# zjykzj/YOLOv4

Hardware: AMD Instinct MI355X
Metric: images/sec fwd+bwd @608x608 bs=64 per GPU (YOLOv4 training step: forward + YOLOLoss + backward) (higher is better)
Workload: dtype f32

## Files before the change

include/yolov4_amd.h:

```cpp
#ifndef YOLOV4_AMD_H
#define YOLOV4_AMD_H

#include <stddef.h>
#include <stdint.h>

#ifdef __cplusplus
extern "C" {
#endif

#define Y4_OK 0
#define Y4_ERR_SHAPE 1
#define Y4_ERR_NULL 2
#define Y4_ERR_LAUNCH 3
#define Y4_ERR_WORKSPACE 4
#define Y4_ERR_NODEVICE 5
#define Y4_ERR_FORMAT 6
#define Y4_ERR_UNSUPPORTED 7

#define Y4_ACT_LINEAR 0
#define Y4_ACT_LEAKY 1
#define Y4_ACT_MISH 2
#define Y4_ACT_RELU 3

const char* y4_strerror(int code);
// ... 75 lines not shown
size_t y4_conv2d_dgrad_workspace(int Cin, int Cout, int k);
int y4_conv2d_dgrad_f32(const float* dy, int lddy, const float* w , float* dx, int lddx,
                        int B, int H, int W, int Cin, int Cout, int k, int stride,
                        void* workspace, size_t workspace_bytes, const unsigned* dy_amax ,
                        const float* residual, int ldr, void* stream);

size_t y4_conv2d_wgrad_workspace(int B, int H, int W, int Cin, int Cout, int k, int stride);
int y4_conv2d_wgrad_f32(const float* x, int ldx, const float* dy, int lddy, float* dw,
                        int B, int H, int W, int Cin, int Cout, int k, int stride,
                        void* workspace, size_t workspace_bytes,
                        const unsigned* x_amax, const unsigned* dy_amax , void* stream);
size_t y4_conv2d_stem_wgrad_workspace(int B, int H, int W, int Cout);
int y4_conv2d_stem_wgrad_f32(const float* x, long long sxb, long long sxc, long long sxh, long long sxw,
                             const float* dy, int lddy, float* dw, int B, int H, int W, int Cout,
                             void* workspace, size_t workspace_bytes, void* stream);

size_t y4_bn_workspace(long long M, int C);
size_t y4_bn_finalize_workspace(int C);
int y4_bn_stats_f32(const float* y, int ldy, long long M, int C, float* mean, float* invstd,
                    float* running_mean, float* running_var, long long* num_batches_tracked,
                    float momentum, float eps, void* workspace, size_t workspace_bytes, void* stream);
int y4_bn_finalize_partials_f32(const float* partials, long long nparts, long long M, int C,
                                float* mean, float* invstd, float* running_mean, float* running_var,
                                long long* num_batches_tracked, float momentum, float eps,
                                void* workspace, size_t workspace_bytes, void* stream);
int y4_bn_planes_bound_f32(const float* gamma, const float* beta, int C, long long M, const unsigned* floor_word, unsigned* out,
                           void* stream);
int y4_bn_act_fwd_f32(const float* y, int ldy, const float* mean, const float* invstd,
                      const float* gamma, const float* beta, int act,
                      const float* residual, int ldr, float* z, int ldz,
// ... 190 lines not shown
```

yolov4_amd/_lib.py:

```python
import ctypes
import os
from ctypes import c_char_p, c_double, c_float, c_int, c_longlong, c_size_t, c_void_p

_HERE = os.path.dirname(os.path.abspath(__file__))
LIB_PATH = os.environ.get('Y4_LIB_PATH') or os.path.join(_HERE, 'lib', 'libyolov4_amd.so')

ACT_IDS = {'linear': 0, 'leaky_relu': 1, 'mish': 2, 'relu': 3}


class Y4Error(RuntimeError):
    pass


P = c_void_p
I, L, F, Z = c_int, c_longlong, c_float, c_size_t

PROTOTYPES = {
    'y4_strerror': (c_char_p, [I]),
    'y4_version': (I, []),
    'y4_device_count': (I, []),
    'y4_set_conv_mode': (I, [I]),
    'y4_get_conv_mode': (I, []),
    'y4_set_planes_bf16': (I, [I]),
    'y4_get_planes_bf16': (I, []),
# ... 13 lines not shown
    'y4_conv2d_fwd_planes_f32': (I, [P, P, P, I, I, I, I, I, I, I, I, P, Z, P, P, P, Z, P, Z, I, P, P]),
    'y4_conv2d_dgrad_planes_f32': (I, [P, P, P, I, I, I, I, I, I, I, I, P, Z, P, P, I, P]),
    'y4_conv2d_wgrad_planes_workspace': (Z, [I, I, I, I, I, I, I]),
    'y4_conv2d_wgrad_planes_f32': (I, [P, P, P, I, I, I, I, I, I, I, P, Z, P, P, P]),
    'y4_conv2d_generic_fwd_f32': (I, [P, I, P, P, I, I, I, I, I, I, I, I, P, P, I, P, I, P]),
    'y4_conv2d_generic_dgrad_f32': (I, [P, I, P, P, I, I, I, I, I, I, I, I, P, I, P]),
    'y4_conv2d_generic_wgrad_f32': (I, [P, I, P, I, P, I, I, I, I, I, I, I, P]),
    'y4_conv2d_stem_dgrad_f32': (I, [P, I, P, P, L, L, L, L, I, I, I, I, P]),
    'y4_conv2d_stem_fwd_f32': (I, [P, L, L, L, L, P, P, I, I, I, I, I, P, P, I, P, P]),
    'y4_conv2d_dgrad_workspace': (Z, [I, I, I]),
    'y4_conv2d_dgrad_f32': (I, [P, I, P, P, I, I, I, I, I, I, I, I, P, Z, P, P, I, P]),
    'y4_conv2d_wgrad_workspace': (Z, [I, I, I, I, I, I, I]),
    'y4_conv2d_wgrad_f32': (I, [P, I, P, I, P, I, I, I, I, I, I, I, P, Z, P, P, P]),
    'y4_conv2d_stem_wgrad_workspace': (Z, [I, I, I, I]),
    'y4_conv2d_stem_wgrad_f32': (I, [P, L, L, L, L, P, I, P, I, I, I, I, P, Z, P]),
    'y4_bn_workspace': (Z, [L, I]),
    'y4_bn_finalize_workspace': (Z, [I]),
    'y4_bn_finalize_partials_f32': (I, [P, L, L, I, P, P, P, P, P, F, F, P, Z, P]),
    'y4_bn_stats_f32': (I, [P, I, L, I, P, P, P, P, P, F, F, P, Z, P]),
    'y4_bn_act_fwd_f32': (I, [P, I, P, P, P, P, I, P, I, P, I, L, I, P, I, P, P, P]),
    'y4_bn_planes_bound_f32': (I, [P, P, I, L, P, P, P]),
    'y4_bn_act_bwd_f32': (I, [P, I, P, I, P, P, P, P, I, P, I, P, P, L, I, P, Z, P, P, P, I, P]),
    'y4_bias_grad_workspace': (Z, [L, I]),
    'y4_bias_grad_f32': (I, [P, I, L, I, P, P, Z, P]),
    'y4_bn_fold_f32': (I, [P, P, P, P, F, P, P, I, P]),
    'y4_copy_channels_f32': (I, [P, I, P, I, L, I, P]),
    'y4_add_f32': (I, [P, I, P, I, P, I, L, I, P]),
    'y4_maxpool_s1_fwd_f32': (I, [P, I, P, I, P, I, I, I, I, I, P]),
    'y4_maxpool_s1_bwd_f32': (I, [P, I, P, P, I, I, I, I, I, I, I, P]),
    'y4_upsample2x_fwd_f32': (I, [P, I, P, I, I, I, I, I, P]),
# ... 110 lines not shown
```

yolov4_amd/csrc/common.h:

```cpp
#pragma once
#include <hip/hip_runtime.h>
#include <stdint.h>
#include "../../include/yolov4_amd.h"

typedef float f32x4 __attribute__((ext_vector_type(4)));
typedef float f32x16 __attribute__((ext_vector_type(16)));
typedef unsigned int u32x4 __attribute__((ext_vector_type(4)));

#define Y4_CHECK_LAUNCH()                                   \
    do {                                                    \
        if (hipGetLastError() != hipSuccess) return Y4_ERR_LAUNCH; \
    } while (0)

static inline hipStream_t y4_stream(void* s) { return reinterpret_cast<hipStream_t>(s); }

#include <atomic>
struct Y4DynLds {
    std::atomic<unsigned long long> done{0ull};
    bool ensure(const void* kernel, size_t bytes) {
        int d = 0;
        if (hipGetDevice(&d) != hipSuccess) return false;
        if (d >= 0 && d < 64 && ((done.load(std::memory_order_acquire) >> d) & 1ull)) return true;
        if (hipFuncSetAttribute(kernel, hipFuncAttributeMaxDynamicSharedMemorySize, (int)bytes) != hipSuccess) return false;
        if (d >= 0 && d < 64) done.fetch_or(1ull << d, std::memory_order_release);
// ... 51 lines not shown
}

__device__ __forceinline__ int y4_xcd_remap(int bid, int nwg) {
    const int q = nwg >> 3, r = nwg & 7, xcd = bid & 7;
    const int base = (xcd < r) ? xcd * (q + 1) : r * (q + 1) + (xcd - r) * q;
    return base + (bid >> 3);
}

__device__ __forceinline__ __amdgpu_buffer_rsrc_t y4_make_rsrc(const void* base, unsigned num_bytes) {
    return __builtin_amdgcn_make_buffer_rsrc(const_cast<void*>(base), (short)0, (int)num_bytes, 0x00020000);
}
__device__ __forceinline__ f32x4 y4_buf_load4(__amdgpu_buffer_rsrc_t r, unsigned voff_bytes, unsigned soff_bytes) {
    const u32x4 v = __builtin_amdgcn_raw_buffer_load_b128(r, (int)voff_bytes, (int)soff_bytes, 0);
    return __builtin_bit_cast(f32x4, v);
}
```

yolov4_amd/csrc/conv_igemm.hip:

```cpp
#include <stdlib.h>
#include "common.h"
#include <cstdarg>
#include <cstdio>
#include "conv_geom.h"

namespace {

constexpr int BK = 32;


using y4::ConvGeom;
using y4::WgradGeom;

template <int BM, int BN, int WM, int WN, bool TRANSPOSED, int BKT = 32>
__global__ __launch_bounds__(256, (BKT == 16 ? 3 : 2)) void conv_gather_mfma_f32(const ConvGeom g) {
    constexpr int LPR = BKT / 4;
    constexpr int RPP = 256 / LPR;
    constexpr int PA = BM / RPP, PB = BN / RPP;
    constexpr int LDS_PITCH = BKT + 4;
    constexpr int BK = BKT;
    constexpr int WTM = BM / WM, WTN = BN / WN;
    constexpr int TM = WTM / 32, TN = WTN / 32;
    static_assert(WM * WN == 4, "4 waves");
    extern __shared__ __attribute__((aligned(16))) float smem[];
// ... 214 lines not shown
        }
        __syncthreads();
        for (int c = tid; c < BN; c += 256) {
            float cs = 0.f, css = 0.f;
#pragma unroll
            for (int w = 0; w < WM; ++w) { cs += red[(w * BN + c) * 2]; css += red[(w * BN + c) * 2 + 1]; }
            const int n = n0 + c;
            if (n < g.N) {
                g.stats[((long long)mt_local * 2 + 0) * g.N + n] = cs;
                g.stats[((long long)mt_local * 2 + 1) * g.N + n] = css;
            }
        }
    }
}

typedef __bf16 bf16x8 __attribute__((ext_vector_type(8)));
typedef unsigned int u32x2 __attribute__((ext_vector_type(2)));

__device__ __forceinline__ unsigned pack_hi16(unsigned x1, unsigned x0) { return __builtin_amdgcn_perm(x1, x0, 0x07060302u); }

__device__ __forceinline__ unsigned rn_bf16_bits(float x) {
    const unsigned u = __float_as_uint(x);
    return u + 0x7fffu + ((u >> 16) & 1u);
}
__device__ __forceinline__ u32x2 round1x4(const f32x4 v) {
    u32x2 p;
    p[0] = pack_hi16(rn_bf16_bits(v[1]), rn_bf16_bits(v[0]));
    p[1] = pack_hi16(rn_bf16_bits(v[3]), rn_bf16_bits(v[2]));
    return p;
}

__device__ __forceinline__ void split3x4(const f32x4 v, u32x2& p1, u32x2& p2, u32x2& p3) {
    unsigned h1[4], h2[4], h3[4];
#pragma unroll
    for (int e = 0; e < 4; ++e) {
        h1[e] = __float_as_uint(v[e]);
        const float r1 = v[e] - __uint_as_float(h1[e] & 0xffff0000u);
        h2[e] = __float_as_uint(r1);
        const float r2 = r1 - __uint_as_float(h2[e] & 0xffff0000u);
        h3[e] = __float_as_uint(r2);
    }
    p1[0] = pack_hi16(h1[1], h1[0]); p1[1] = pack_hi16(h1[3], h1[2]);
    p2[0] = pack_hi16(h2[1], h2[0]); p2[1] = pack_hi16(h2[3], h2[2]);
    p3[0] = pack_hi16(h3[1], h3[0]); p3[1] = pack_hi16(h3[3], h3[2]);
}

template <int BM, int BN, int WM, int WN, bool TRANSPOSED, int NP = 3>
__global__ __launch_bounds__(256, 2) void conv_gather_bf16x3(const ConvGeom g) {
    constexpr int BK = 32;
    constexpr int PITCH_B = 80;
    constexpr int PA = BM / 32;
    constexpr int NB = (BN * 4 + 255) / 256;
    constexpr int WTM = BM / WM, WTN = BN / WN;
    constexpr int TM = WTM / 32, TN = WTN / 32;
    static_assert(WM * WN == 4, "4 waves");
    extern __shared__ __attribute__((aligned(16))) unsigned char smem_b[];
    unsigned char* As = smem_b;
    unsigned char* Bs = smem_b + NP * BM * PITCH_B;
    int* row_m = reinterpret_cast<int*>(smem_b + NP * (BM + BN) * PITCH_B);
// ... 1288 lines not shown
__global__ __launch_bounds__(256) void stem_wgrad_reduce2_kernel(const double* __restrict__ part, float* __restrict__ dw,
                                                                 int nparts, int Cout) {
    for (int i = threadIdx.x; i < Cout * 27; i += 256) {
        const int n = i / 27, j = i - n * 27;
        double s = 0.0;
        for (int k = 0; k < nparts; ++k) s += part[(long long)k * 1024 + n * 32 + j];
        dw[i] = (float)s;
    }
}

constexpr int STEM_WAVES = 4096;

}

namespace y4 {
int slab_reduce(const float* slabs, float* dw, long long n, int splits, hipStream_t st) {
    if ((n & 3) == 0 && !(reinterpret_cast<uintptr_t>(dw) & 15) && !(reinterpret_cast<uintptr_t>(slabs) & 15)) {
        const long long nvec = n / 4;
        if (nvec >= 64 * 1024)
            hipLaunchKernelGGL(slab_reduce_vec_kernel<64>, dim3((unsigned)((nvec + 63) / 64)), dim3(256), 0, st,
                               reinterpret_cast<const f32x4*>(slabs), reinterpret_cast<f32x4*>(dw), nvec, splits);
        else
            hipLaunchKernelGGL(slab_reduce_vec_kernel<16>, dim3((unsigned)((nvec + 15) / 16)), dim3(256), 0, st,
                               reinterpret_cast<const f32x4*>(slabs), reinterpret_cast<f32x4*>(dw), nvec, splits);
    } else {
        const int blocks = (int)((n + 255) / 256 > 2048 ? 2048 : (n + 255) / 256);
        hipLaunchKernelGGL(slab_reduce_kernel, dim3(blocks), dim3(256), 0, st, slabs, dw, n, splits);
    }
    Y4_CHECK_LAUNCH();
    return Y4_OK;
// ... 381 lines not shown
```

yolov4_amd/csrc/pointwise.hip:

```cpp
#include "common.h"

namespace {

constexpr int PW_THREADS = 256;
constexpr int PW_UNROLL = 4;
#define Y4_ACT_SWITCH(ACTV, CALL)                                              \
    switch (ACTV) {                                                            \
        case Y4_ACT_MISH: { constexpr int A_ = Y4_ACT_MISH; CALL; } break;     \
        case Y4_ACT_LEAKY: { constexpr int A_ = Y4_ACT_LEAKY; CALL; } break;   \
        case Y4_ACT_RELU: { constexpr int A_ = Y4_ACT_RELU; CALL; } break;     \
        default: { constexpr int A_ = Y4_ACT_LINEAR; CALL; } break;            \
    }

struct RowMap {
    int tpr;
    int rpb;
};
static inline RowMap row_map(int C) {
    RowMap r;
    int c4 = C / 4;
    r.tpr = c4 < PW_THREADS ? c4 : PW_THREADS;
    int p = 1;
    while (p * 2 <= r.tpr) p *= 2;
    r.tpr = p;
// ... 132 lines not shown
    if (blockIdx.x == 0 && threadIdx.x == 0 && nbt) *nbt += 1;
    const int c = blockIdx.x * 32 + (threadIdx.x & 31);
    if ((threadIdx.x >> 5) != 0 || c >= C) return;
    const double mu = s / (double)M;
    double var = ss / (double)M - mu * mu;
    if (var < 0) var = 0;
    mean[c] = (float)mu;
    invstd[c] = (float)(1.0 / sqrt(var + (double)eps));
    if (rmean) rmean[c] = (1.0f - momentum) * rmean[c] + momentum * (float)mu;
    if (rvar) {
        const double unb = M > 1 ? var * (double)M / (double)(M - 1) : var;
        rvar[c] = (1.0f - momentum) * rvar[c] + momentum * (float)unb;
    }
}

__device__ __forceinline__ void amax_track(unsigned& m, const f32x4 o) {
#pragma unroll
    for (int e = 0; e < 4; ++e) {
        const unsigned b = __float_as_uint(o[e]) & 0x7fffffffu;
        if (b < 0x7f800000u && b > m) m = b;
    }
}
__device__ __forceinline__ void amax_commit(unsigned m, unsigned* out) {
    __shared__ unsigned wmax[PW_THREADS / 64];
#pragma unroll
    for (int off = 32; off > 0; off >>= 1) {
        const unsigned o = (unsigned)__shfl_xor((int)m, off, 64);
        m = o > m ? o : m;
    }
    if ((threadIdx.x & 63) == 0) wmax[threadIdx.x >> 6] = m;
    __syncthreads();
    if (threadIdx.x == 0) {
        unsigned v = wmax[0];
#pragma unroll
        for (int w = 1; w < PW_THREADS / 64; ++w) v = wmax[w] > v ? wmax[w] : v;
        if (v > __hip_atomic_load(out, __ATOMIC_RELAXED, __HIP_MEMORY_SCOPE_AGENT)) atomicMax(out, v);
    }
}

__global__ __launch_bounds__(256) void bn_planes_bound_kernel(const float* __restrict__ gamma, const float* __restrict__ beta, int C,
                                                              float sqrt_m1, const unsigned* __restrict__ res_amax,
                                                              unsigned* __restrict__ out, const unsigned* __restrict__ floor_word = nullptr) {
    __shared__ float red[256];
    float m = 0.f;
    for (int c = threadIdx.x; c < C; c += 256) m = fmaxf(m, fabsf(gamma[c]) * sqrt_m1 + fabsf(beta[c]));
    red[threadIdx.x] = m;
    __syncthreads();
    for (int s = 128; s > 0; s >>= 1) {
        if (threadIdx.x < s) red[threadIdx.x] = fmaxf(red[threadIdx.x], red[threadIdx.x + s]);
        __syncthreads();
    }
    if (threadIdx.x == 0) {
        float b = red[0] * 1.0001f;
// ... 944 lines not shown
    if (n <= 0 || act < 0 || act > 3) return Y4_ERR_SHAPE;
    hipLaunchKernelGGL(act_fwd_flat_kernel, dim3(grid_for((n + 3) / 4)), dim3(PW_THREADS), 0, y4_stream(stream), x, y, n, act);
    Y4_CHECK_LAUNCH();
    return Y4_OK;
}

int y4_act_bwd_f32(const float* x, const float* dy, float* dx, long long n, int act, void* stream) {
    if (!x || !dy || !dx) return Y4_ERR_NULL;
    if (n <= 0 || act < 0 || act > 3) return Y4_ERR_SHAPE;
    hipLaunchKernelGGL(act_bwd_flat_kernel, dim3(grid_for((n + 3) / 4)), dim3(PW_THREADS), 0, y4_stream(stream), x, dy, dx, n, act);
    Y4_CHECK_LAUNCH();
    return Y4_OK;
}

}
```

yolov4_amd/ops.py:

```python
import ctypes
import functools
import os

import torch

from ._lib import ACT_IDS, Y4Error, check, float_array, int_array, lib

CL = torch.channels_last


def _stream():
    return ctypes.c_void_p(torch.cuda.current_stream().cuda_stream)


def _ptr(t):
    return ctypes.c_void_p(t.data_ptr()) if t is not None else None


def _require_gpu(t, what):
    if not t.is_cuda:
        raise Y4Error(f'{what}: tensor is on {t.device}; the yolov4_amd hot path runs on an MI355X only '
                      '(no CPU fallback)')
    if t.dtype != torch.float32:
        raise Y4Error(f'{what}: expected float32, got {t.dtype}')
# ... 263 lines not shown
        nbytes = L.y4_conv2d_fwd_workspace(Cin, Cout, k)
        cws = _ws(nbytes, x.device)
        check(L.y4_conv2d_fwd_bnstats_f32(_ptr(x), ldx, _ptr(w), _ptr(y), ldy, B, H, W, Cin, Cout, k, s,
                                          _ptr(part), pbytes, ctypes.byref(n), _ptr(x_amax), _ptr(cws), nbytes,
                                          _ptr(dgrad_filter), dgrad_filter.numel() if dgrad_filter is not None else 0, _stream()),
              'conv2d_fwd_bnstats')
        nparts = n.value
    mean = torch.empty(Cout, device=x.device, dtype=torch.float32)
    invstd = torch.empty(Cout, device=x.device, dtype=torch.float32)
    wsb = L.y4_bn_finalize_workspace(Cout)
    ws = _ws(wsb, x.device)
    check(L.y4_bn_finalize_partials_f32(_ptr(part), nparts, B * Ho * Wo, Cout, _ptr(mean), _ptr(invstd),
                                        _ptr(running_mean), _ptr(running_var), _ptr(nbt), float(momentum), float(eps),
                                        _ptr(ws), wsb, _stream()), 'bn_finalize_partials')
    return y, mean, invstd


class Planes:
    __slots__ = ('buf', 'shape', 'amax')

    def __init__(self, buf, shape, amax):
        self.buf, self.shape, self.amax = buf, tuple(shape), amax


class PlanesTensor(torch.Tensor):
    __torch_function__ = torch._C._disabled_torch_function_impl

    def _refuse(self, *a, **kw):
        raise Y4Error('this tensor holds a PRE-SPLIT activation (two fp16 pieces per element, csrc/conv_planes.hip), not '
                      'float32 values: only ConvBNAct can consume it.  Register the forward hook before the forward pass '
# ... 455 lines not shown
        if xp is not None:
            x_amax = xp.amax
        elif f16 and x_amax is None and (ctx.needs_input_grad[0] or ctx.needs_input_grad[1]):
            x_amax = amax_raw(x)
        ctx.x_amax = x_amax
        if bn and training:
            if x.shape[0] * conv_out_hw(x.shape[2], x.shape[3], k, s)[0] * conv_out_hw(x.shape[2], x.shape[3], k, s)[1] <= 1:
                raise ValueError('Expected more than 1 value per channel when training')
            ctx.dgrad_filter = None
            if ((f16 or (bfm and xp is not None)) and ctx.needs_input_grad[0] and x.shape[1] % 32 == 0 and fast_conv_shape(x.shape[1], k, s)
                    and weight.shape[0] % 4 == 0 and (xp is None or weight.shape[0] % 32 == 0)
                    and not (bfm and xp is not None and s == 2
                             and not s2_plane_dgrad(x.shape[0], x.shape[2], x.shape[3], x.shape[1], weight.shape[0]))):
                ctx.dgrad_filter = dgrad_filter_buffer(x.shape[1], weight.shape[0], k, x.device)
            ybf = ctx.y_bf16 = bool(bfm and xp is not None and weight.shape[0] % 32 == 0 and _BF16_Y)
            if xp is not None:
                y, mean, invstd = conv_fwd_planes_bnstats_raw(xp, weight, k, s, cfg['running_mean'], cfg['running_var'],
                                                              cfg['nbt'], cfg['momentum'], cfg['eps'], dgrad_filter=ctx.dgrad_filter,
                                                              y_bf16=ybf)
            else:
                y, mean, invstd = conv_fwd_bnstats_raw(x, weight, k, s, cfg['running_mean'], cfg['running_var'],
                                                       cfg['nbt'], cfg['momentum'], cfg['eps'], x_amax=x_amax,
                                                       dgrad_filter=ctx.dgrad_filter)
            want = cfg.get('out_planes')
            cb = cfg.get('out_cat')
            if cb is not None and cb.planes:
                z = bn_act_fwd_raw(y, mean, invstd, gamma, beta, act, residual, out=dest, planes='slot', y_bf16=ybf)
                if io is not None:
                    io['z_planes'] = True
                z_amax = cb.cell[0:1] if cb.cell is not None else None
# ... 63 lines not shown
            else:
                ctx.save_for_backward(x, weight)
                ctx.mode = 'nobn_linear'
        if io is not None:
            io['z_amax'] = z_amax
        return z

    @staticmethod
    def backward(ctx, dz):
        cfg = ctx.cfg
        k, s, act = cfg['k'], cfg['s'], cfg['act']
        f16 = f16x2_mode() and ctx.x_shape[1] != 3
        dy_amax = dy_pl = dyP = wq = None
        x_amax = live(ctx.x_amax)
        x_planes = getattr(ctx, 'x_planes', False)
        if ctx.mode in ('bn_train', 'bn_eval_grad'):
            x, weight, y, mean, invstd, gamma, beta = ctx.saved_tensors
            gp, bp = cfg.get('gamma_param'), cfg.get('beta_param')
            sink = (gp is not None and bp is not None and getattr(gp, '_y4_grad_fresh', False)
                    and getattr(bp, '_y4_grad_fresh', False) and gp.grad is not None and bp.grad is not None
                    and ctx.needs_input_grad[3] and ctx.needs_input_grad[4])
            bfp = x_planes and planes_mode() == 'bf16'
            planes = planes_cell(dz.device, 8) if (x_planes and not bfp) else None
            dy_amax = planes[5:6] if planes is not None else (new_amax(dz.device) if f16 else None)
            twin_dy = x_planes and s == 2 and ctx.needs_input_grad[0] and not s2_plane_dgrad(
                ctx.x_shape[0], ctx.x_shape[2], ctx.x_shape[3], ctx.x_shape[1], dz.shape[1])
            res = bn_act_bwd_raw(dz, y, mean, invstd, gamma, beta, act,
                                 gp.grad if sink else None, bp.grad if sink else None,
                                 out_amax=None if planes is not None else dy_amax, planes=planes,
                                 frozen=ctx.mode == 'bn_eval_grad', bf16=bfp, twin=twin_dy, y_bf16=getattr(ctx, 'y_bf16', False))
# ... 731 lines not shown
```

Measured before the change: 449.0.

## Fuse stem conv with BatchNorm and activation via recompute in fwd and bwd

Adds a dedicated stem path (3-channel 3x3 stride-1 conv) that runs the conv with bf16x3 split MFMA, first to compute BN statistics and then again to apply BN+activation and write z directly, so the pre-BN y tensor is never stored. The backward pass recomputes the conv output to get BN/activation gradients and fuses the weight gradient into the same pass, with no dgrad since the input needs no gradient. This removes a full-resolution read and write of y at 608x608 with 32 channels. The cost is doing the conv two or three times, plus new kernels and several extra small reduction launches.

```diff
diff --git a/include/yolov4_amd.h b/include/yolov4_amd.h
--- a/include/yolov4_amd.h
+++ b/include/yolov4_amd.h
@@ -113,6 +113,19 @@
 int y4_conv2d_stem_wgrad_f32(const float* x, long long sxb, long long sxc, long long sxh, long long sxw,
                              const float* dy, int lddy, float* dw, int B, int H, int W, int Cout,
                              void* workspace, size_t workspace_bytes, void* stream);
+
+int y4_stem_fused_ok(long long sxb, long long sxc, long long sxh, long long sxw, int B, int H, int W, int Cout);
+size_t y4_stem_bn_act_fwd_workspace(int B, int H, int W, int Cout);
+int y4_stem_bn_act_fwd_f32(const float* x, long long sxb, long long sxc, long long sxh, long long sxw, const float* w,
+                           int B, int H, int W, int Cout, const float* gamma, const float* beta, int act,
+                           float* mean, float* invstd, float* running_mean, float* running_var, long long* num_batches_tracked,
+                           float momentum, float eps, float* z, int ldz, unsigned* out_amax,
+                           void* workspace, size_t workspace_bytes, void* stream);
+size_t y4_stem_bn_act_bwd_workspace(int B, int H, int W, int Cout);
+int y4_stem_bn_act_bwd_f32(const float* x, long long sxb, long long sxc, long long sxh, long long sxw, const float* w,
+                           const float* dz, int lddz, const float* mean, const float* invstd, const float* gamma,
+                           const float* beta, int act, int B, int H, int W, int Cout,
+                           float* dgamma, float* dbeta, float* dw, void* workspace, size_t workspace_bytes, void* stream);
 
 size_t y4_bn_workspace(long long M, int C);
 size_t y4_bn_finalize_workspace(int C);
diff --git a/yolov4_amd/_lib.py b/yolov4_amd/_lib.py
--- a/yolov4_amd/_lib.py
+++ b/yolov4_amd/_lib.py
@@ -51,6 +51,11 @@
     'y4_conv2d_wgrad_f32': (I, [P, I, P, I, P, I, I, I, I, I, I, I, P, Z, P, P, P]),
     'y4_conv2d_stem_wgrad_workspace': (Z, [I, I, I, I]),
     'y4_conv2d_stem_wgrad_f32': (I, [P, L, L, L, L, P, I, P, I, I, I, I, P, Z, P]),
+    'y4_stem_fused_ok': (I, [L, L, L, L, I, I, I, I]),
+    'y4_stem_bn_act_fwd_workspace': (Z, [I, I, I, I]),
+    'y4_stem_bn_act_fwd_f32': (I, [P, L, L, L, L, P, I, I, I, I, P, P, I, P, P, P, P, P, F, F, P, I, P, P, Z, P]),
+    'y4_stem_bn_act_bwd_workspace': (Z, [I, I, I, I]),
+    'y4_stem_bn_act_bwd_f32': (I, [P, L, L, L, L, P, P, I, P, P, P, P, I, I, I, I, I, P, P, P, P, Z, P]),
     'y4_bn_workspace': (Z, [L, I]),
     'y4_bn_finalize_workspace': (Z, [I]),
     'y4_bn_finalize_partials_f32': (I, [P, L, L, I, P, P, P, P, P, F, F, P, Z, P]),
diff --git a/yolov4_amd/csrc/common.h b/yolov4_amd/csrc/common.h
--- a/yolov4_amd/csrc/common.h
+++ b/yolov4_amd/csrc/common.h
@@ -89,3 +89,52 @@
     const u32x4 v = __builtin_amdgcn_raw_buffer_load_b128(r, (int)voff_bytes, (int)soff_bytes, 0);
     return __builtin_bit_cast(f32x4, v);
 }
+
+typedef __bf16 bf16x8 __attribute__((ext_vector_type(8)));
+typedef unsigned int u32x2 __attribute__((ext_vector_type(2)));
+__device__ __forceinline__ unsigned pack_hi16(unsigned x1, unsigned x0) { return __builtin_amdgcn_perm(x1, x0, 0x07060302u); }
+__device__ __forceinline__ void split3x4(const f32x4 v, u32x2& p1, u32x2& p2, u32x2& p3) {
+    unsigned h1[4], h2[4], h3[4];
+#pragma unroll
+    for (int e = 0; e < 4; ++e) {
+        h1[e] = __float_as_uint(v[e]);
+        const float r1 = v[e] - __uint_as_float(h1[e] & 0xffff0000u);
+        h2[e] = __float_as_uint(r1);
+        const float r2 = r1 - __uint_as_float(h2[e] & 0xffff0000u);
+        h3[e] = __float_as_uint(r2);
+    }
+    p1[0] = pack_hi16(h1[1], h1[0]); p1[1] = pack_hi16(h1[3], h1[2]);
+    p2[0] = pack_hi16(h2[1], h2[0]); p2[1] = pack_hi16(h2[3], h2[2]);
+    p3[0] = pack_hi16(h3[1], h3[0]); p3[1] = pack_hi16(h3[3], h3[2]);
+}
+
+__device__ __forceinline__ void amax_track1(unsigned& m, const float o) {
+    const unsigned b = __float_as_uint(o) & 0x7fffffffu;
+    if (b < 0x7f800000u && b > m) m = b;
+}
+__device__ __forceinline__ void amax_track(unsigned& m, const f32x4 o) {
+#pragma unroll
+    for (int e = 0; e < 4; ++e) amax_track1(m, o[e]);
+}
+__device__ __forceinline__ void amax_commit(unsigned m, unsigned* out) {
+    __shared__ unsigned wmax[4];
+#pragma unroll
+    for (int off = 32; off > 0; off >>= 1) {
+        const unsigned o = (unsigned)__shfl_xor((int)m, off, 64);
+        m = o > m ? o : m;
+    }
+    if ((threadIdx.x & 63) == 0) wmax[threadIdx.x >> 6] = m;
+    __syncthreads();
+    if (threadIdx.x == 0) {
+        unsigned v = wmax[0];
+#pragma unroll
+        for (int w = 1; w < 4; ++w) v = wmax[w] > v ? wmax[w] : v;
+        if (v > __hip_atomic_load(out, __ATOMIC_RELAXED, __HIP_MEMORY_SCOPE_AGENT)) atomicMax(out, v);
+    }
+}
+
+namespace y4 {
+int bn_bwd_fold_finalize(const float* part, long long nparts, long long M, int C, void* workspace, float* dgamma, float* dbeta,
+                         const float* gamma, const float* invstd, hipStream_t st);
+int stem_wgrad_fold(const float* slabs, int nslabs, double* part, float* dw, int Cout, hipStream_t st);
+}
diff --git a/yolov4_amd/csrc/conv_igemm.hip b/yolov4_amd/csrc/conv_igemm.hip
--- a/yolov4_amd/csrc/conv_igemm.hip
+++ b/yolov4_amd/csrc/conv_igemm.hip
@@ -252,10 +252,6 @@
     }
 }
 
-typedef __bf16 bf16x8 __attribute__((ext_vector_type(8)));
-typedef unsigned int u32x2 __attribute__((ext_vector_type(2)));
-
-__device__ __forceinline__ unsigned pack_hi16(unsigned x1, unsigned x0) { return __builtin_amdgcn_perm(x1, x0, 0x07060302u); }
 
 __device__ __forceinline__ unsigned rn_bf16_bits(float x) {
     const unsigned u = __float_as_uint(x);
@@ -266,21 +262,6 @@
     p[0] = pack_hi16(rn_bf16_bits(v[1]), rn_bf16_bits(v[0]));
     p[1] = pack_hi16(rn_bf16_bits(v[3]), rn_bf16_bits(v[2]));
     return p;
-}
-
-__device__ __forceinline__ void split3x4(const f32x4 v, u32x2& p1, u32x2& p2, u32x2& p3) {
-    unsigned h1[4], h2[4], h3[4];
-#pragma unroll
-    for (int e = 0; e < 4; ++e) {
-        h1[e] = __float_as_uint(v[e]);
-        const float r1 = v[e] - __uint_as_float(h1[e] & 0xffff0000u);
-        h2[e] = __float_as_uint(r1);
-        const float r2 = r1 - __uint_as_float(h2[e] & 0xffff0000u);
-        h3[e] = __float_as_uint(r2);
-    }
-    p1[0] = pack_hi16(h1[1], h1[0]); p1[1] = pack_hi16(h1[3], h1[2]);
-    p2[0] = pack_hi16(h2[1], h2[0]); p2[1] = pack_hi16(h2[3], h2[2]);
-    p3[0] = pack_hi16(h3[1], h3[0]); p3[1] = pack_hi16(h3[3], h3[2]);
 }
 
 template <int BM, int BN, int WM, int WN, bool TRANSPOSED, int NP = 3>
@@ -1599,6 +1580,13 @@
 }
 
 namespace y4 {
+int stem_wgrad_fold(const float* slabs, int nslabs, double* part, float* dw, int Cout, hipStream_t st) {
+    hipLaunchKernelGGL(stem_wgrad_reduce1_kernel, dim3(64), dim3(256), 0, st, slabs, part, nslabs);
+    Y4_CHECK_LAUNCH();
+    hipLaunchKernelGGL(stem_wgrad_reduce2_kernel, dim3(1), dim3(256), 0, st, part, dw, 64, Cout);
+    Y4_CHECK_LAUNCH();
+    return Y4_OK;
+}
 int slab_reduce(const float* slabs, float* dw, long long n, int splits, hipStream_t st) {
     if ((n & 3) == 0 && !(reinterpret_cast<uintptr_t>(dw) & 15) && !(reinterpret_cast<uintptr_t>(slabs) & 15)) {
         const long long nvec = n / 4;
diff --git a/yolov4_amd/csrc/pointwise.hip b/yolov4_amd/csrc/pointwise.hip
--- a/yolov4_amd/csrc/pointwise.hip
+++ b/yolov4_amd/csrc/pointwise.hip
@@ -170,29 +170,6 @@
     }
 }
 
-__device__ __forceinline__ void amax_track(unsigned& m, const f32x4 o) {
-#pragma unroll
-    for (int e = 0; e < 4; ++e) {
-        const unsigned b = __float_as_uint(o[e]) & 0x7fffffffu;
-        if (b < 0x7f800000u && b > m) m = b;
-    }
-}
-__device__ __forceinline__ void amax_commit(unsigned m, unsigned* out) {
-    __shared__ unsigned wmax[PW_THREADS / 64];
-#pragma unroll
-    for (int off = 32; off > 0; off >>= 1) {
-        const unsigned o = (unsigned)__shfl_xor((int)m, off, 64);
-        m = o > m ? o : m;
-    }
-    if ((threadIdx.x & 63) == 0) wmax[threadIdx.x >> 6] = m;
-    __syncthreads();
-    if (threadIdx.x == 0) {
-        unsigned v = wmax[0];
-#pragma unroll
-        for (int w = 1; w < PW_THREADS / 64; ++w) v = wmax[w] > v ? wmax[w] : v;
-        if (v > __hip_atomic_load(out, __ATOMIC_RELAXED, __HIP_MEMORY_SCOPE_AGENT)) atomicMax(out, v);
-    }
-}
 
 __global__ __launch_bounds__(256) void bn_planes_bound_kernel(const float* __restrict__ gamma, const float* __restrict__ beta, int C,
                                                               float sqrt_m1, const unsigned* __restrict__ res_amax,
@@ -1167,3 +1144,18 @@
 }
 
 }
+
+namespace y4 {
+int bn_bwd_fold_finalize(const float* part, long long nparts, long long M, int C, void* workspace, float* dgamma, float* dbeta,
+                         const float* gamma, const float* invstd, hipStream_t st) {
+    double* acc = static_cast<double*>(workspace);
+    double* bacc = acc + 2 * C;
+    int nb = 0;
+    const int rc = fold_partials(part, nparts, C, bacc, &nb, st);
+    if (rc != Y4_OK) return rc;
+    hipLaunchKernelGGL(bn_bwd_finalize_kernel, dim3((C + 31) / 32), dim3(256), 0, st, bacc, nb, C, acc, dgamma, dbeta, gamma,
+                       invstd, 1.0 / (double)M, static_cast<unsigned*>(nullptr));
+    Y4_CHECK_LAUNCH();
+    return Y4_OK;
+}
+}
diff --git a/yolov4_amd/csrc/stem_fused.hip b/yolov4_amd/csrc/stem_fused.hip
--- /dev/null
+++ b/yolov4_amd/csrc/stem_fused.hip
@@ -0,0 +1,423 @@
+#include "conv_geom.h"
+
+namespace {
+
+struct StemFusedGeom {
+    const float* x; const float* w;
+    long long sxb, sxc, sxh, sxw;
+    int B, H, W, Cout;
+    long long M;
+    int ngroups;
+    float inv_hw, inv_w;
+    const float* mean; const float* invstd; const float* gamma; const float* beta;
+    float* stats;
+    float* z; long long ldz; unsigned* out_amax;
+    const float* dz; long long lddz;
+    float* part;
+    const double* acc; double invM;
+    float* slabs;
+};
+
+struct StemBody {
+    bf16x8 fb[2][3];
+    int koff[16];
+    int ktap[16];
+    __amdgpu_buffer_rsrc_t rsrc;
+
+    __device__ __forceinline__ void init(const StemFusedGeom& g, int fr, int fh) {
+#pragma unroll
+        for (int i = 0; i < 16; ++i) {
+            const int k = (i >> 3) * 16 + fh * 8 + (i & 7);
+            const int r = k / 9, c = (k - r * 9) / 3, q = k - r * 9 - c * 3;
+            const bool kv = k < 27;
+            koff[i] = kv ? (int)(c * g.sxc + (r - 1) * g.sxh + (q - 1) * g.sxw) * 4 : 0;
+            ktap[i] = kv ? r * 3 + q : 9;
+        }
+#pragma unroll
+        for (int ks = 0; ks < 2; ++ks) {
+            f32x4 w0, w1;
+#pragma unroll
+            for (int i = 0; i < 8; ++i) {
+                const int k = ks * 16 + fh * 8 + i;
+                const int r = k / 9, c = (k - r * 9) / 3, q = k - r * 9 - c * 3;
+                const float v = (k < 27 && fr < g.Cout) ? g.w[fr * 27 + (r * 3 + q) * 3 + c] : 0.f;
+                if (i < 4) w0[i] = v; else w1[i - 4] = v;
+            }
+            u32x2 a1, a2, a3, b1, b2, b3;
+            split3x4(w0, a1, a2, a3);
+            split3x4(w1, b1, b2, b3);
+            const u32x4 q1 = {a1[0], a1[1], b1[0], b1[1]}, q2 = {a2[0], a2[1], b2[0], b2[1]}, q3 = {a3[0], a3[1], b3[0], b3[1]};
+            fb[ks][0] = __builtin_bit_cast(bf16x8, q1); fb[ks][1] = __builtin_bit_cast(bf16x8, q2); fb[ks][2] = __builtin_bit_cast(bf16x8, q3);
+        }
+        rsrc = y4_make_rsrc(g.x, 0xfffffff0u);
+    }
+
+    static __device__ __forceinline__ void coords(const StemFusedGeom& g, long long p, int& b, int& h, int& w) {
+        const int HW = g.H * g.W;
+        b = (int)((float)p * g.inv_hw);
+        int rem = (int)(p - (long long)b * HW);
+        if (rem < 0) { --b; rem += HW; } else if (rem >= HW) { ++b; rem -= HW; }
+        h = (int)((float)rem * g.inv_w);
+        w = rem - h * g.W;
+        if (w < 0) { --h; w += g.W; } else if (w >= g.W) { ++h; w -= g.W; }
+    }
+
+    __device__ __forceinline__ void load(const StemFusedGeom& g, float (&xv)[16], long long tile, int fr) const {
+        const long long p = tile * 32 + fr;
+        unsigned base = 0xffffffffu;
+        unsigned m9 = 0;
+        if (p < g.M) {
+            int b, h, w;
+            coords(g, p, b, h, w);
+            base = (unsigned)(b * g.sxb + h * g.sxh + w * g.sxw) * 4u;
+            const unsigned hm = (h > 0 ? 1u : 0u) | 2u | (h + 1 < g.H ? 4u : 0u);
+            const unsigned wm = (w > 0 ? 1u : 0u) | 2u | (w + 1 < g.W ? 4u : 0u);
+            m9 = ((hm & 1u) ? wm : 0u) | ((hm & 2u) ? wm << 3 : 0u) | ((hm & 4u) ? wm << 6 : 0u);
+        }
+#pragma unroll
+        for (int i = 0; i < 16; ++i) {
+            const bool ok = (m9 >> ktap[i]) & 1u;
+            xv[i] = __builtin_bit_cast(float, __builtin_amdgcn_raw_buffer_load_b32(rsrc, ok ? (int)(base + (unsigned)koff[i]) : -1, 0, 0));
+        }
+    }
+
+    __device__ __forceinline__ f32x16 mma(const float (&xv)[16]) const {
+        f32x16 acc;
+#pragma unroll
+        for (int e = 0; e < 16; ++e) acc[e] = 0.f;
+#pragma unroll
+        for (int ks = 0; ks < 2; ++ks) {
+            const f32x4 v0 = {xv[ks * 8 + 0], xv[ks * 8 + 1], xv[ks * 8 + 2], xv[ks * 8 + 3]};
+            const f32x4 v1 = {xv[ks * 8 + 4], xv[ks * 8 + 5], xv[ks * 8 + 6], xv[ks * 8 + 7]};
+            u32x2 a1, a2, a3, b1, b2, b3;
+            split3x4(v0, a1, a2, a3);
+            split3x4(v1, b1, b2, b3);
+            const u32x4 q1 = {a1[0], a1[1], b1[0], b1[1]}, q2 = {a2[0], a2[1], b2[0], b2[1]}, q3 = {a3[0], a3[1], b3[0], b3[1]};
+            const bf16x8 f1 = __builtin_bit_cast(bf16x8, q1), f2 = __builtin_bit_cast(bf16x8, q2), f3 = __builtin_bit_cast(bf16x8, q3);
+            acc = __builtin_amdgcn_mfma_f32_32x32x16_bf16(f3, fb[ks][0], acc, 0, 0, 0);
+            acc = __builtin_amdgcn_mfma_f32_32x32x16_bf16(f2, fb[ks][1], acc, 0, 0, 0);
+            acc = __builtin_amdgcn_mfma_f32_32x32x16_bf16(f1, fb[ks][2], acc, 0, 0, 0);
+            acc = __builtin_amdgcn_mfma_f32_32x32x16_bf16(f2, fb[ks][0], acc, 0, 0, 0);
+            acc = __builtin_amdgcn_mfma_f32_32x32x16_bf16(f1, fb[ks][1], acc, 0, 0, 0);
+            acc = __builtin_amdgcn_mfma_f32_32x32x16_bf16(f1, fb[ks][0], acc, 0, 0, 0);
+        }
+        return acc;
+    }
+};
+
+__device__ __forceinline__ int acc_row(int e, int fh) { return 4 * fh + (e & 3) + 8 * (e >> 2); }
+
+struct GroupWindow {
+    __amdgpu_buffer_rsrc_t rs;
+    __device__ __forceinline__ GroupWindow(const float* t, long long ld, int Cout, long long p0, long long M) {
+        const long long rows = M - p0 < 256 ? M - p0 : 256;
+        rs = y4_make_rsrc(t + p0 * ld, (unsigned)(((rows - 1) * ld + Cout) * 4));
+    }
+};
+__device__ __forceinline__ int win_off(int row, long long ld, int fr, bool cok) {
+    return cok ? (int)(((unsigned)row * (unsigned)ld + (unsigned)fr) * 4u) : -1;
+}
+
+__device__ __forceinline__ float square_rounded(float v) {
+#pragma clang fp contract(off)
+    return v * v;
+}
+
+__global__ __launch_bounds__(256) void stem_bn_stats_kernel(const StemFusedGeom g) {
+    __shared__ float sred[4][32][2];
+    const int tid = threadIdx.x, lane = tid & 63, wave = tid >> 6;
+    const int fr = lane & 31, fh = lane >> 5;
+    StemBody body;
+    body.init(g, fr, fh);
+    float xv0[16], xv1[16];
+    for (int grp = blockIdx.x; grp < g.ngroups; grp += gridDim.x) {
+        const long long t0 = (long long)grp * 8 + wave * 2;
+        body.load(g, xv0, t0, fr);
+        body.load(g, xv1, t0 + 1, fr);
+        float cs = 0.f, css = 0.f;
+        {
+            const f32x16 acc = body.mma(xv0);
+#pragma unroll
+            for (int e = 0; e < 16; ++e) { const float raw = acc[e]; cs += raw; css += square_rounded(raw); }
+        }
+        {
+            const f32x16 acc = body.mma(xv1);
+#pragma unroll
+            for (int e = 0; e < 16; ++e) { const float raw = acc[e]; cs += raw; css += square_rounded(raw); }
+        }
+        cs += __shfl_xor(cs, 32, 64);
+        css += __shfl_xor(css, 32, 64);
+        if (fh == 0) { sred[wave][fr][0] = cs; sred[wave][fr][1] = css; }
+        __syncthreads();
+        if (tid < 64) {
+            const int c = tid & 31, which = tid >> 5;
+            const float t = (sred[0][c][which] + sred[1][c][which]) + (sred[2][c][which] + sred[3][c][which]);
+            if (c < g.Cout) g.stats[((long long)grp * 2 + which) * g.Cout + c] = t;
+        }
+        __syncthreads();
+    }
+}
+
+template <int ACT>
+__global__ __launch_bounds__(256, 3) void stem_bn_act_write_kernel(const StemFusedGeom g) {
+    const int tid = threadIdx.x, lane = tid & 63, wave = tid >> 6;
+    const int fr = lane & 31, fh = lane >> 5;
+    const bool cok = fr < g.Cout;
+    StemBody body;
+    body.init(g, fr, fh);
+    const float a = cok ? g.invstd[fr] * g.gamma[fr] : 0.f;
+    const float b = cok ? g.beta[fr] - g.mean[fr] * a : 0.f;
+    unsigned amax = 0u;
+    float xv0[16], xv1[16];
+    for (int grp = blockIdx.x; grp < g.ngroups; grp += gridDim.x) {
+        const long long p0 = (long long)grp * 256;
+        const long long t0 = (long long)grp * 8 + wave * 2;
+        const GroupWindow zw(g.z, g.ldz, g.Cout, p0, g.M);
+        const int rows = (int)(g.M - p0 < 256 ? g.M - p0 : 256);
+        body.load(g, xv0, t0, fr);
+        body.load(g, xv1, t0 + 1, fr);
+        auto emit = [&](const f32x16 acc, int row0) {
+#pragma unroll
+            for (int e = 0; e < 16; ++e) {
+                const int row = row0 + acc_row(e, fh);
+                const float o = y4_act_t<ACT>(acc[e] * a + b);
+                __builtin_amdgcn_raw_buffer_store_b32(__float_as_uint(o), zw.rs, win_off(row, g.ldz, fr, cok), 0, 0);
+                if (cok && row < rows) amax_track1(amax, o);
+            }
+        };
+        emit(body.mma(xv0), wave * 64);
+        emit(body.mma(xv1), wave * 64 + 32);
+    }
+    if (g.out_amax) amax_commit(amax, g.out_amax);
+}
+
+struct BnLane {
+    float mu, is, ga, be;
+    __device__ __forceinline__ BnLane(const StemFusedGeom& g, int fr, bool cok) {
+        mu = cok ? g.mean[fr] : 0.f; is = cok ? g.invstd[fr] : 0.f; ga = cok ? g.gamma[fr] : 0.f; be = cok ? g.beta[fr] : 0.f;
+    }
+};
+
+__device__ __forceinline__ void load_dz(const GroupWindow& dw, const StemFusedGeom& g, float (&d)[16], int row0, int fr, int fh, bool cok) {
+#pragma unroll
+    for (int e = 0; e < 16; ++e)
+        d[e] = __builtin_bit_cast(float, __builtin_amdgcn_raw_buffer_load_b32(dw.rs, win_off(row0 + acc_row(e, fh), g.lddz, fr, cok), 0, 0));
+}
+
+template <int ACT>
+__global__ __launch_bounds__(256, 3) void stem_bn_bwd_reduce_kernel(const StemFusedGeom g) {
+    __shared__ float sred[4][32][2];
+    const int tid = threadIdx.x, lane = tid & 63, wave = tid >> 6;
+    const int fr = lane & 31, fh = lane >> 5;
+    const bool cok = fr < g.Cout;
+    StemBody body;
+    body.init(g, fr, fh);
+    const BnLane bn(g, fr, cok);
+    float S = 0.f, SX = 0.f;
+    float xv0[16], xv1[16], d0[16], d1[16];
+    for (int grp = blockIdx.x; grp < g.ngroups; grp += gridDim.x) {
+        const long long p0 = (long long)grp * 256;
+        const long long t0 = (long long)grp * 8 + wave * 2;
+        const GroupWindow dw(g.dz, g.lddz, g.Cout, p0, g.M);
+        body.load(g, xv0, t0, fr);
+        body.load(g, xv1, t0 + 1, fr);
+        load_dz(dw, g, d0, wave * 64, fr, fh, cok);
+        load_dz(dw, g, d1, wave * 64 + 32, fr, fh, cok);
+        float s = 0.f, sx = 0.f;
+        auto add = [&](const f32x16 acc, const float (&d)[16]) {
+#pragma unroll
+            for (int e = 0; e < 16; ++e) {
+                const float xh = (acc[e] - bn.mu) * bn.is;
+                const float gq = d[e] * y4_act_grad_t<ACT>(bn.ga * xh + bn.be);
+                s += gq;
+                sx += gq * xh;
+            }
+        };
+        add(body.mma(xv0), d0);
+        add(body.mma(xv1), d1);
+        S += s; SX += sx;
+    }
+    S += __shfl_xor(S, 32, 64);
+    SX += __shfl_xor(SX, 32, 64);
+    if (fh == 0) { sred[wave][fr][0] = S; sred[wave][fr][1] = SX; }
+    __syncthreads();
+    if (tid < 64) {
+        const int c = tid & 31, which = tid >> 5;
+        const float t = (sred[0][c][which] + sred[1][c][which]) + (sred[2][c][which] + sred[3][c][which]);
+        if (c < g.Cout) g.part[((long long)blockIdx.x * 2 + which) * g.Cout + c] = t;
+    }
+}
+
+template <int ACT>
+__global__ __launch_bounds__(256, 2) void stem_bn_bwd_apply_wgrad_kernel(const StemFusedGeom g) {
+    const int tid = threadIdx.x, lane = tid & 63, wave = tid >> 6;
+    const int fr = lane & 31, fh = lane >> 5;
+    const bool cok = fr < g.Cout;
+    StemBody body;
+    body.init(g, fr, fh);
+    const BnLane bn(g, fr, cok);
+    const float k1 = cok ? (float)(g.acc[fr] * g.invM) : 0.f;
+    const float k2 = cok ? (float)(g.acc[g.Cout + fr] * g.invM) : 0.f;
+    const float gi = bn.ga * bn.is;
+    const bool jok = fr < 27;
+    const int tap = jok ? fr / 3 : 0, cj = jok ? fr - tap * 3 : 0;
+    const int rj = tap / 3 - 1, qj = tap - (tap / 3) * 3 - 1;
+    const unsigned joff = (unsigned)(cj * g.sxc + rj * g.sxh + qj * g.sxw);
+    f32x16 wacc;
+#pragma unroll
+    for (int e = 0; e < 16; ++e) wacc[e] = 0.f;
+    auto load_b = [&](float (&bv)[16], long long tile) {
+        long long p = tile * 32 + 4 * fh;
+        int b = 0, h = 0, w = 0;
+        if (p < g.M) StemBody::coords(g, p, b, h, w);
+#pragma unroll
+        for (int e = 0; e < 16; ++e) {
+            const int hi = h + rj, wi = w + qj;
+            const bool ok = jok && p < g.M && (unsigned)hi < (unsigned)g.H && (unsigned)wi < (unsigned)g.W;
+            const unsigned xo = ((unsigned)(b * g.sxb + h * g.sxh + w * g.sxw) + joff) * 4u;
+            bv[e] = __builtin_bit_cast(float, __builtin_amdgcn_raw_buffer_load_b32(body.rsrc, ok ? (int)xo : -1, 0, 0));
+            const int d = (e & 3) == 3 ? 5 : 1;
+            p += d;
+            w += d;
+            if (w >= g.W) { w -= g.W; if (++h == g.H) { h = 0; ++b; } }
+        }
+    };
+    float xv0[16], xv1[16], d[16], bv[16];
+    for (int grp = blockIdx.x; grp < g.ngroups; grp += gridDim.x) {
+        const long long p0 = (long long)grp * 256;
+        const long long t0 = (long long)grp * 8 + wave * 2;
+        const GroupWindow dw(g.dz, g.lddz, g.Cout, p0, g.M);
+        const int rows = (int)(g.M - p0 < 256 ? g.M - p0 : 256);
+        body.load(g, xv0, t0, fr);
+        body.load(g, xv1, t0 + 1, fr);
+        load_dz(dw, g, d, wave * 64, fr, fh, cok);
+        load_b(bv, t0);
+        auto fold = [&](const f32x16 acc, int row0) {
+#pragma unroll
+            for (int e = 0; e < 16; ++e) {
+                const float xh = (acc[e] - bn.mu) * bn.is;
+                const float gq = d[e] * y4_act_grad_t<ACT>(bn.ga * xh + bn.be);
+                float dy = gi * (gq - k1 - xh * k2);
+                if (row0 + acc_row(e, fh) >= rows) dy = 0.f;
+                wacc = __builtin_amdgcn_mfma_f32_32x32x2f32(dy, bv[e], wacc, 0, 0, 0);
+            }
+        };
+        fold(body.mma(xv0), wave * 64);
+        load_dz(dw, g, d, wave * 64 + 32, fr, fh, cok);
+        load_b(bv, t0 + 1);
+        fold(body.mma(xv1), wave * 64 + 32);
+    }
+    float* out = g.slabs + ((long long)blockIdx.x * 4 + wave) * 1024;
+#pragma unroll
+    for (int e = 0; e < 16; ++e) out[acc_row(e, fh) * 32 + fr] = wacc[e];
+}
+
+constexpr int STATS_GRID = 2048;
+constexpr int WGRAD_GRID = 1024;
+
+bool fill_geom(StemFusedGeom& g, const float* x, long long sxb, long long sxc, long long sxh, long long sxw, const float* w,
+               int B, int H, int W, int Cout) {
+    if (!y4_stem_fused_ok(sxb, sxc, sxh, sxw, B, H, W, Cout)) return false;
+    g.x = x; g.w = w; g.sxb = sxb; g.sxc = sxc; g.sxh = sxh; g.sxw = sxw;
+    g.B = B; g.H = H; g.W = W; g.Cout = Cout;
+    g.M = (long long)B * H * W;
+    g.ngroups = (int)((g.M + 255) / 256);
+    g.inv_hw = 1.0f / (float)((long long)H * W);
+    g.inv_w = 1.0f / (float)W;
+    return true;
+}
+bool pitch_ok(int ld, int Cout) { return ld >= Cout && ld < (1 << 21); }
+size_t align256(size_t n) { return (n + 255) & ~(size_t)255; }
+size_t stats_bytes(long long M, int Cout) { return align256((size_t)((M + 255) / 256) * 2 * Cout * sizeof(float)); }
+
+#define Y4_STEM_ACT_SWITCH(ACTV, CALL)                                         \
+    switch (ACTV) {                                                            \
+        case Y4_ACT_MISH: { constexpr int A_ = Y4_ACT_MISH; CALL; } break;     \
+        case Y4_ACT_LEAKY: { constexpr int A_ = Y4_ACT_LEAKY; CALL; } break;   \
+        case Y4_ACT_RELU: { constexpr int A_ = Y4_ACT_RELU; CALL; } break;     \
+        default: { constexpr int A_ = Y4_ACT_LINEAR; CALL; } break;            \
+    }
+
+}
+
+extern "C" {
+
+int y4_stem_fused_ok(long long sxb, long long sxc, long long sxh, long long sxw, int B, int H, int W, int Cout) {
+    const int mode = y4_get_conv_mode();
+    if (mode < 1 || mode > 3) return 0;
+    if (B <= 0 || H <= 0 || W < 5 || Cout <= 0 || Cout > 32 || (Cout & 3)) return 0;
+    if (sxb < 0 || sxc < 0 || sxh < 0 || sxw < 0) return 0;
+    if ((long long)H * W >= (1 << 24)) return 0;
+    if (((long long)B * H * W + 255) / 256 >= (1ll << 31)) return 0;
+    return ((long long)(B - 1) * sxb + 2 * sxc + (long long)(H - 1) * sxh + (long long)(W - 1) * sxw + 1) * 4 < 0xfffffff0ll;
+}
+
+size_t y4_stem_bn_act_fwd_workspace(int B, int H, int W, int Cout) {
+    if (B <= 0 || H <= 0 || W <= 0 || Cout <= 0) return 0;
+    return stats_bytes((long long)B * H * W, Cout) + y4_bn_finalize_workspace(Cout);
+}
+
+int y4_stem_bn_act_fwd_f32(const float* x, long long sxb, long long sxc, long long sxh, long long sxw, const float* w,
+                           int B, int H, int W, int Cout, const float* gamma, const float* beta, int act,
+                           float* mean, float* invstd, float* running_mean, float* running_var, long long* num_batches_tracked,
+                           float momentum, float eps, float* z, int ldz, unsigned* out_amax,
+                           void* workspace, size_t workspace_bytes, void* stream) {
+    if (!x || !w || !gamma || !beta || !mean || !invstd || !z || !workspace) return Y4_ERR_NULL;
+    StemFusedGeom g{};
+    if (!fill_geom(g, x, sxb, sxc, sxh, sxw, w, B, H, W, Cout) || !pitch_ok(ldz, Cout)) return Y4_ERR_SHAPE;
+    if (workspace_bytes < y4_stem_bn_act_fwd_workspace(B, H, W, Cout)) return Y4_ERR_WORKSPACE;
+    hipStream_t st = y4_stream(stream);
+    g.stats = static_cast<float*>(workspace);
+    void* fin = static_cast<char*>(workspace) + stats_bytes(g.M, Cout);
+    const int grid = g.ngroups < STATS_GRID ? g.ngroups : STATS_GRID;
+    hipLaunchKernelGGL(stem_bn_stats_kernel, dim3(grid), dim3(256), 0, st, g);
+    Y4_CHECK_LAUNCH();
+    const int rc = y4_bn_finalize_partials_f32(g.stats, g.ngroups, g.M, Cout, mean, invstd, running_mean, running_var,
+                                               num_batches_tracked, momentum, eps, fin, y4_bn_finalize_workspace(Cout), stream);
+    if (rc != Y4_OK) return rc;
+    g.mean = mean; g.invstd = invstd; g.gamma = gamma; g.beta = beta;
+    g.z = z; g.ldz = ldz; g.out_amax = out_amax;
+    Y4_STEM_ACT_SWITCH(act, hipLaunchKernelGGL(stem_bn_act_write_kernel<A_>, dim3(grid), dim3(256), 0, st, g));
+    Y4_CHECK_LAUNCH();
+    y4::note_kernel("stem_bn_act_write_kernel<%d>", act);
+    return Y4_OK;
+}
+
+size_t y4_stem_bn_act_bwd_workspace(int B, int H, int W, int Cout) {
+    if (B <= 0 || H <= 0 || W <= 0 || Cout <= 0) return 0;
+    return align256(y4_bn_finalize_workspace(Cout)) + align256((size_t)STATS_GRID * 2 * Cout * sizeof(float)) +
+           (size_t)WGRAD_GRID * 4 * 1024 * sizeof(float) + 64 * 1024 * sizeof(double);
+}
+
+int y4_stem_bn_act_bwd_f32(const float* x, long long sxb, long long sxc, long long sxh, long long sxw, const float* w,
+                           const float* dz, int lddz, const float* mean, const float* invstd, const float* gamma,
+                           const float* beta, int act, int B, int H, int W, int Cout,
+                           float* dgamma, float* dbeta, float* dw, void* workspace, size_t workspace_bytes, void* stream) {
+    if (!x || !w || !dz || !mean || !invstd || !gamma || !beta || !dgamma || !dbeta || !dw || !workspace) return Y4_ERR_NULL;
+    StemFusedGeom g{};
+    if (!fill_geom(g, x, sxb, sxc, sxh, sxw, w, B, H, W, Cout) || !pitch_ok(lddz, Cout)) return Y4_ERR_SHAPE;
+    if (workspace_bytes < y4_stem_bn_act_bwd_workspace(B, H, W, Cout)) return Y4_ERR_WORKSPACE;
+    hipStream_t st = y4_stream(stream);
+    char* ws = static_cast<char*>(workspace);
+    void* fin = ws;
+    g.part = reinterpret_cast<float*>(ws + align256(y4_bn_finalize_workspace(Cout)));
+    g.slabs = reinterpret_cast<float*>(reinterpret_cast<char*>(g.part) + align256((size_t)STATS_GRID * 2 * Cout * sizeof(float)));
+    double* wpart = reinterpret_cast<double*>(g.slabs + (size_t)WGRAD_GRID * 4 * 1024);
+    g.mean = mean; g.invstd = invstd; g.gamma = gamma; g.beta = beta;
+    g.dz = dz; g.lddz = lddz;
+    g.acc = static_cast<const double*>(fin); g.invM = 1.0 / (double)g.M;
+    const int rgrid = g.ngroups < STATS_GRID ? g.ngroups : STATS_GRID;
+    Y4_STEM_ACT_SWITCH(act, hipLaunchKernelGGL(stem_bn_bwd_reduce_kernel<A_>, dim3(rgrid), dim3(256), 0, st, g));
+    Y4_CHECK_LAUNCH();
+    int rc = y4::bn_bwd_fold_finalize(g.part, rgrid, g.M, Cout, fin, dgamma, dbeta, gamma, invstd, st);
+    if (rc != Y4_OK) return rc;
+    const int wgrid = g.ngroups < WGRAD_GRID ? g.ngroups : WGRAD_GRID;
+    Y4_STEM_ACT_SWITCH(act, hipLaunchKernelGGL(stem_bn_bwd_apply_wgrad_kernel<A_>, dim3(wgrid), dim3(256), 0, st, g));
+    Y4_CHECK_LAUNCH();
+    rc = y4::stem_wgrad_fold(g.slabs, wgrid * 4, wpart, dw, Cout, st);
+    if (rc != Y4_OK) return rc;
+    y4::note_kernel("stem_bn_bwd_apply_wgrad_kernel<%d>", act);
+    return Y4_OK;
+}
+
+}
diff --git a/yolov4_amd/ops.py b/yolov4_amd/ops.py
--- a/yolov4_amd/ops.py
+++ b/yolov4_amd/ops.py
@@ -301,6 +301,53 @@
                                         _ptr(running_mean), _ptr(running_var), _ptr(nbt), float(momentum), float(eps),
                                         _ptr(ws), wsb, _stream()), 'bn_finalize_partials')
     return y, mean, invstd
+
+
+def stem_fused_ok(x, Cout, k, s):
+    if x.dim() != 4 or x.shape[1] != 3 or k != 3 or s != 1 or x.dtype != torch.float32:
+        return False
+    B, _, H, W = x.shape
+    return bool(lib().y4_stem_fused_ok(*x.stride(), B, H, W, Cout))
+
+
+def stem_bn_act_fwd_raw(x, w, gamma, beta, act, running_mean, running_var, nbt, momentum, eps, out=None, out_amax=None):
+    L = lib()
+    B, _, H, W = x.shape
+    Cout = w.shape[0]
+    z = out if _slot_ok(out, (B, Cout, H, W)) else empty_nhwc(B, Cout, H, W, x.device)
+    mean = torch.empty(Cout, device=x.device, dtype=torch.float32)
+    invstd = torch.empty(Cout, device=x.device, dtype=torch.float32)
+    nbytes = L.y4_stem_bn_act_fwd_workspace(B, H, W, Cout)
+    ws = _ws(nbytes, x.device)
+    check(L.y4_stem_bn_act_fwd_f32(_ptr(x), *x.stride(), _ptr(krsc(w)), B, H, W, Cout, _ptr(gamma), _ptr(beta), ACT_IDS[act],
+                                   _ptr(mean), _ptr(invstd), _ptr(running_mean), _ptr(running_var), _ptr(nbt), float(momentum),
+                                   float(eps), _ptr(z), nhwc_pitch(z), _ptr(out_amax), _ptr(ws), nbytes, _stream()),
+          'stem_bn_act_fwd')
+    return z, mean, invstd
+
+
+def stem_bn_act_bwd_raw(x, w, dz, mean, invstd, gamma, beta, act, dgamma_out=None, dbeta_out=None, dw_out=None):
+    L = lib()
+    B, _, H, W = x.shape
+    Cout = w.shape[0]
+    dz, lddz = as_nhwc(dz, need_vec4=False)
+
+    def slot(t):
+        ok = t is not None and t.dtype == torch.float32 and tuple(t.shape) == (Cout,) and t.is_contiguous() and t.is_cuda
+        return t if ok else torch.empty(Cout, device=x.device, dtype=torch.float32)
+    dgamma, dbeta = slot(dgamma_out), slot(dbeta_out)
+    if dw_out is not None and tuple(dw_out.shape) == tuple(w.shape) and _is_krsc_dense(dw_out):
+        dw = dw_out
+        WGRAD_STATS['in_place'] += 1
+    else:
+        WGRAD_STATS['temporary'] += 1
+        dw = krsc(torch.empty(tuple(w.shape), device=x.device, dtype=torch.float32).contiguous(memory_format=CL))
+    nbytes = L.y4_stem_bn_act_bwd_workspace(B, H, W, Cout)
+    ws = _ws(nbytes, x.device)
+    check(L.y4_stem_bn_act_bwd_f32(_ptr(x), *x.stride(), _ptr(krsc(w)), _ptr(dz), lddz, _ptr(mean), _ptr(invstd), _ptr(gamma),
+                                   _ptr(beta), ACT_IDS[act], B, H, W, Cout, _ptr(dgamma), _ptr(dbeta), _ptr(dw),
+                                   _ptr(ws), nbytes, _stream()), 'stem_bn_act_bwd')
+    return dw, dgamma, dbeta
 
 
 class Planes:
@@ -786,6 +833,20 @@
                              and not s2_plane_dgrad(x.shape[0], x.shape[2], x.shape[3], x.shape[1], weight.shape[0]))):
                 ctx.dgrad_filter = dgrad_filter_buffer(x.shape[1], weight.shape[0], k, x.device)
             ybf = ctx.y_bf16 = bool(bfm and xp is not None and weight.shape[0] % 32 == 0 and _BF16_Y)
+            cb = cfg.get('out_cat')
+            if (xp is None and residual is None and not cfg.get('out_planes') and not (cb is not None and cb.planes)
+                    and not ctx.needs_input_grad[0] and stem_fused_ok(x, weight.shape[0], k, s)):
+                if f16x2_mode():
+                    z_amax = live(cfg.get('out_amax')) if (dest is not None and _slot_ok(dest, (x.shape[0], weight.shape[0]) + tuple(x.shape[2:]))) else None
+                    if z_amax is None:
+                        z_amax = new_amax(x.device)
+                z, mean, invstd = stem_bn_act_fwd_raw(x, weight, gamma, beta, act, cfg['running_mean'], cfg['running_var'],
+                                                      cfg['nbt'], cfg['momentum'], cfg['eps'], out=dest, out_amax=z_amax)
+                ctx.save_for_backward(x, weight, mean, invstd, gamma, beta)
+                ctx.mode = 'stem_fused'
+                if io is not None:
+                    io['z_amax'] = z_amax
+                return z
             if xp is not None:
                 y, mean, invstd = conv_fwd_planes_bnstats_raw(xp, weight, k, s, cfg['running_mean'], cfg['running_var'],
                                                               cfg['nbt'], cfg['momentum'], cfg['eps'], dgrad_filter=ctx.dgrad_filter,
@@ -879,6 +940,29 @@
         dy_amax = dy_pl = dyP = wq = None
         x_amax = live(ctx.x_amax)
         x_planes = getattr(ctx, 'x_planes', False)
+        if ctx.mode == 'stem_fused':
+            x, weight, mean, invstd, gamma, beta = ctx.saved_tensors
+            gp, bp, wp = cfg.get('gamma_param'), cfg.get('beta_param'), cfg.get('weight_param')
+
+            def fresh(p):
+                return p is not None and getattr(p, '_y4_grad_fresh', False) and p.grad is not None
+            sink = fresh(gp) and fresh(bp) and ctx.needs_input_grad[3] and ctx.needs_input_grad[4]
+            wsink = fresh(wp) and ctx.needs_input_grad[1]
+            dw, dgamma, dbeta = stem_bn_act_bwd_raw(x, weight, dz, mean, invstd, gamma, beta, act,
+                                                    gp.grad if sink else None, bp.grad if sink else None,
+                                                    wp.grad if wsink else None)
+            if sink and dgamma is gp.grad and dbeta is bp.grad:
+                gp._y4_grad_fresh = bp._y4_grad_fresh = False
+                gp._y4_grad_ready()
+                bp._y4_grad_ready()
+                dgamma = dbeta = None
+            if wsink:
+                wp._y4_grad_fresh = False
+                if dw is not wp.grad:
+                    wp.grad.add_(dw)
+                wp._y4_grad_ready()
+                dw = None
+            return None, dw if ctx.needs_input_grad[1] else None, None, dgamma, dbeta, None, None
         if ctx.mode in ('bn_train', 'bn_eval_grad'):
             x, weight, y, mean, invstd, gamma, beta = ctx.saved_tensors
             gp, bp = cfg.get('gamma_param'), cfg.get('beta_param')
```

New measurement: 453.5 (median of 6 runs). 1.01x the previous value.
